# archi-physics/archi

Measured on AMD Instinct MI355X. Metric: kNN queries/sec @ top-10, 10M x 768 bf16 corpus, higher is better.
Workload: dtype bf16

## Files before the change

### archi_amd/csrc/index.hip

```cpp
#include "index.h"
#include "switches.h"

#include <algorithm>
#include <atomic>
#include <cmath>
#include <cstring>
#include <limits>
#include <chrono>
#include <dlfcn.h>
#include <unordered_set>

namespace ak {

static thread_local std::string g_err;
void set_error(const std::string &msg) { g_err = msg; }

extern "C" char **environ;
static const std::unordered_map<std::string, std::string> &env_snapshot() {
    static const std::unordered_map<std::string, std::string> *snap = [] {
        auto *m = new std::unordered_map<std::string, std::string>();
        for (char **e = environ; e && *e; e++) {
            if (strncmp(*e, "AK_", 3) != 0) continue;
            const char *eq = strchr(*e, '=');
            if (eq) (*m)[std::string(*e, (size_t)(eq - *e))] = std::string(eq + 1);
        }
        return m;
    }();
    return *snap;
}
const char *env_get(const char *name) {
    const auto &m = env_snapshot();
    const auto it = m.find(name);
    return it == m.end() ? nullptr : it->second.c_str();
}
int env_int(const char *name, int dflt) {
    const char *e = env_get(name);
    return e && *e ? atoi(e) : dflt;
}
namespace {
struct SwitchName { const char *name; std::atomic<int> Switches::*field; int dflt; bool is_flag; bool wrong_results; bool is_char; };
const SwitchName g_switch_names[] = {
    {"AK_SCAN_CFG", &Switches::scan_cfg, 0, false, false, true},
    {"AK_SCAN_MFMA", &Switches::scan_mfma, 0, false, false, false},
    {"AK_SCAN_I8", &Switches::scan_i8, AK_SCAN_I8_DEFAULT, false, false, false},
    {"AK_SCAN_BLOCKS", &Switches::scan_blocks, 0, false, false, false},
    {"AK_SCAN_NO192", &Switches::scan_no192, 0, true, false, false},
    {"AK_SEED_RATIO", &Switches::seed_ratio, 32, false, false, false},
    {"AK_SEED_DIV", &Switches::seed_div, 0, false, false, false},
    {"AK_PRE_DIV", &Switches::pre_div, 0, false, false, false},
    {"AK_SCAN_NOSEED", &Switches::scan_noseed, 0, true, false, false},
    {"AK_SCAN_NOPRE", &Switches::scan_nopre, 0, true, false, false},
    {"AK_TAIL_OLD", &Switches::tail_old, 0, true, false, false},
    {"AK_RERANK_OLD", &Switches::rerank_old, 0, false, false, false},
    {"AK_SCAN_DBG", &Switches::scan_dbg, 0, true, false, false},
    {"AK_COALESCE_STATS", &Switches::coalesce_stats, 0, true, false, false},
    {"AK_COALESCE", &Switches::coalesce, 1, false, false, false},
    {"AK_LEX_BATCH_PAIRS", &Switches::lex_batch_pairs, 1 << 24, false, false, false},
    {"AK_LEX_BATCH_TERMS", &Switches::lex_batch_terms, 0, false, false, false},
    {"AK_SHARD_INJECT", &Switches::shard_inject, 0, false, false, false},
    {"AK_QUERY_FUSED", &Switches::query_fused, 0, false, false, false},
#if AK_DBG_KERNELS
    {"AK_SCAN_ABLATE", &Switches::scan_ablate, 0, false, true, false},
    {"AK_TAIL_ABLATE", &Switches::tail_ablate, 0, false, true, false},
#endif
};
int switch_value(const SwitchName &n, const char *v) {
    if (!v || !*v) return n.dflt;
    if (n.is_char) return (int)(unsigned char)v[0];
    if (n.is_flag) return 1;
    return atoi(v);
}
}
Switches &switches() {
    static Switches sw;
    static const bool once = [] {
        for (const SwitchName &n : g_switch_names) {
            if (n.wrong_results && !DBG_KERNELS) continue;
            (sw.*(n.field)).store(switch_value(n, env_get(n.name)), std::memory_order_relaxed);
        }
        if (const char *e = env_get("AK_SCAN_R192")) sw.scan_r192_pm.store((int)(atof(e) * 1000.0 + 0.5), std::memory_order_relaxed);
        return true;
    }();
    (void)once;
    return sw;
}
__attribute__((constructor)) static void ak_read_environment_at_load() { (void)switches(); }
int switches_set(const char *name, const char *value) {
    if (!name) return -1;
    Switches &sw = switches();
    if (!strcmp(name, "AK_SCAN_R192")) {
        sw.scan_r192_pm.store(value && *value ? (int)(atof(value) * 1000.0 + 0.5) : 850, std::memory_order_relaxed);
        return 0;
    }
    for (const SwitchName &n : g_switch_names)
        if (!strcmp(name, n.name)) {
            if (n.wrong_results && !DBG_KERNELS) return -1;
            if (!DBG_KERNELS && n.is_char && value && (*value == 'X' || *value == 'O')) return -1;
            if (!DBG_KERNELS && n.field == &Switches::scan_mfma && switch_value(n, value) != 0) return -1;
            if (n.field == &Switches::scan_mfma && switch_value(n, value) != 0 && switch_value(n, value) != 16 && switch_value(n, value) != 32) return -1;
            (sw.*(n.field)).store(switch_value(n, value), std::memory_order_relaxed);
            return 0;
        }
    return -1;
}

namespace {
struct RoctxApi {
    int (*push)(const char *) = nullptr;
    int (*pop)() = nullptr;
    RoctxApi() {
        for (const char *lib : {"librocprofiler-sdk-roctx.so.1", "librocprofiler-sdk-roctx.so", "libroctx64.so.4", "libroctx64.so"}) {
            if (void *h = dlopen(lib, RTLD_NOW | RTLD_GLOBAL)) {
                push = (int (*)(const char *))dlsym(h, "roctxRangePushA");
                pop = (int (*)())dlsym(h, "roctxRangePop");
                if (push && pop) return;
                push = nullptr; pop = nullptr;
            }
        }
    }
};
const RoctxApi &roctx() {
    static const RoctxApi api;
    return api;
}
}
RoctxRange::RoctxRange(const char *name) : on(roctx().push != nullptr) { if (on) roctx().push(name); }
RoctxRange::~RoctxRange() { if (on) roctx().pop(); }

int Workspace::reserve(size_t need) {
    if (need <= bytes) return 0;
    if (buf) hipFree(buf);
    buf = nullptr; bytes = 0;
    AK_HIP(hipMalloc(&buf, need));
    bytes = need;
    return 0;
}
void Workspace::release() {
    if (buf) hipFree(buf);
    buf = nullptr; bytes = 0;
}

constexpr size_t SCRATCH_KEEP = 256ull << 20;
struct ThreadCtx {
    hipStream_t stream = nullptr;
    char *dev = nullptr; size_t dev_cap = 0;
    char *ws = nullptr; size_t ws_cap = 0;
    char *pin = nullptr; size_t pin_cap = 0;
    void trim() {
        if (dev_cap > SCRATCH_KEEP) { hipFree(dev); dev = nullptr; dev_cap = 0; }
        if (ws_cap > SCRATCH_KEEP) { hipFree(ws); ws = nullptr; ws_cap = 0; }
        if (pin_cap > SCRATCH_KEEP) { hipHostFree(pin); pin = nullptr; pin_cap = 0; }
    }
// ... 1235 lines not shown
```

### archi_amd/csrc/scan.hip

```cpp
#include <atomic>
#include "index.h"
#include "switches.h"
#include "mfma_tile.h"

#include <type_traits>

namespace ak {
using namespace mt;

constexpr int BK = 64;

__device__ inline uint64_t ld_sc1(const uint64_t *p) { return __builtin_nontemporal_load(p); }

__device__ inline float max3f(float a, float b, float c) {
    float r;
    asm("v_max3_f32 %0, %1, %2, %3" : "=v"(r) : "v"(a), "v"(b), "v"(c));
    return r;
}
__device__ inline float max3z(float a, float b) {
    float r;
    asm("v_max3_f32 %0, %1, %2, 0" : "=v"(r) : "v"(a), "v"(b));
    return r;
}

// ... 67 lines not shown

template <int NS>
__device__ __noinline__ int compact_impl(uint64_t *buf, int m, int k, int limit, float mar, int lane,
                                          float *thr_io, int *cnt_out, int *trig_out, int trig_max,
                                          uint64_t *final_out ) {
    uint64_t key[NS];
#pragma unroll
    for (int j = 0; j < NS; j++) {
        const int idx = j * 64 + lane;
        key[j] = idx < m ? ld_sc1(buf + idx) : KEY_INVALID;
    }
    float thr = *thr_io;
    if (m >= k) {
        const uint64_t tk = kth_key<NS>(key, k);
        const float t = key_score((uint32_t)(tk >> 32)) - mar;
        if (t > thr) thr = t;
    }
    uint64_t cut = ((uint64_t)score_key(thr) << 32) | 0xffffffffull;
    int c = 0;
#pragma unroll
    for (int j = 0; j < NS; j++) c += __popcll(__ballot(key[j] != KEY_INVALID && key[j] <= cut));
    if (c > limit) cut = kth_key<NS>(key, limit);
    uint64_t *dst = final_out ? final_out : buf;
    int run = 0;
#pragma unroll
    for (int j = 0; j < NS; j++) {
        const bool keep = key[j] != KEY_INVALID && key[j] <= cut;
        const uint64_t mask = __ballot(keep);
        const int pos = run + __popcll(mask & ((1ull << lane) - 1ull));
        if (keep) dst[pos] = key[j];
        run += __popcll(mask);
    }
    if (final_out) {
        for (int i = run + lane; i < limit; i += 64) final_out[i] = KEY_INVALID;
    } else if (lane == 0) {
        *cnt_out = run;
        const int tr = 2 * run > 64 ? 2 * run : 64;
        *trig_out = tr < trig_max ? tr : trig_max;
    }
    if (lane == 0) *thr_io = thr;
    return run;
}

template <int CAP>
__device__ inline int compact_wave(uint64_t *buf, int m, int k, int limit, float mar, int lane, float *thr_io,
                                    int *cnt_out, int *trig_out, int trig_max, uint64_t *final_out) {
    if (m <= 64) return compact_impl<1>(buf, m, k, limit, mar, lane, thr_io, cnt_out, trig_out, trig_max, final_out);
    else if (m <= 128) return compact_impl<2>(buf, m, k, limit, mar, lane, thr_io, cnt_out, trig_out, trig_max, final_out);
    else if (m <= 256) return compact_impl<4>(buf, m, k, limit, mar, lane, thr_io, cnt_out, trig_out, trig_max, final_out);
    else if (CAP >= 512 && m <= 512) return compact_impl<8>(buf, m, k, limit, mar, lane, thr_io, cnt_out, trig_out, trig_max, final_out);
    else return compact_impl<CAP / 64>(buf, m, k, limit, mar, lane, thr_io, cnt_out, trig_out, trig_max, final_out);
}

template <int WM_, int WN_, int MI_, int NI_, int NSTAGE_, int MINW_, bool PHASED_ = false, int MFMA_ = 32>
struct ScanCfg {
    static constexpr int WM = WM_, WN = WN_, MI = MI_, NI = NI_, NSTAGE = NSTAGE_, MINW = MINW_;
    static constexpr bool PHASED = PHASED_;
    static constexpr int MFMA = MFMA_;
    static constexpr bool I8 = false;
    using Shape32 = ScanCfg<WM_, WN_, MI_, NI_, NSTAGE_, MINW_, PHASED_, 32>;
    static_assert(MFMA_ == 32 || (MFMA_ == 16 && PHASED_), "the 16x16x32 shape exists for the phased tiles");
    static constexpr int AHEAD = NSTAGE_ - 1;
    static constexpr int BKB = 128;
    static constexpr int RPP = 1024 / BKB;
    static constexpr int CPR = BKB / 16;
    static constexpr int NSUB = BKB / 32;
    static constexpr int NW = WM * WN;
    static constexpr int THREADS = NW * 64;
    static constexpr int BM = WM * MI * 32;
    static constexpr int BN = WN * NI * 32;
    static constexpr int A_BYTES = BM * BKB, B_BYTES = BN * BKB;
    static constexpr int A_PW = BM / RPP / NW;
    static constexpr int B_PW = BN / RPP / NW;
    static constexpr int LOADS = A_PW + B_PW;
    static constexpr int CAP = BM >= 256 ? 1024 : 512;
    static constexpr int LDS_BYTES = NSTAGE * (A_BYTES + B_BYTES) + (4 * BM + 4 * BN + 4 + 128) * 4;
    static constexpr bool SEED_GM_LDS = PHASED_ && MI_ * NI_ >= 8;
    static constexpr int SEED_LDS_BYTES = LDS_BYTES + (SEED_GM_LDS ? NW * MI_ * NI_ * 64 * 4 : 0);
    static_assert(SEED_LDS_BYTES <= 160 * 1024, "LDS budget");
    static_assert((BM / RPP) % NW == 0 && (BN / RPP) % NW == 0, "pieces must divide over the waves");
    static_assert(NSTAGE >= 2 && NSTAGE <= 4, "ring depth");
    static_assert(BM / 64 <= NW, "ea/eb staging uses one wave per 64 rows");
    static_assert(!PHASED_ || (NSTAGE_ == 2 && ((WM_ == 2 && WN_ == 4 && MI_ == 4 && (NI_ == 2 || NI_ == 1)) ||
                                                 (WM_ == 4 && WN_ == 2 && MI_ == 2 && NI_ == 3))),
                  "phased K-loop: 256 x 256 / 256 x 128 tile (8 waves of 128 x 64 / 128 x 32) or 256 x 192 (8 waves of 64 x 96), two K-tile buffers");
};

template <bool IS_BF16, class C, bool SEED, bool INSTR, bool SEEDPASS = false>
__global__ __launch_bounds__(C::THREADS, C::MINW) void k_scan(
    const uint16_t *__restrict__ rows, const float *__restrict__ ea, const float *__restrict__ eb,
    const float *__restrict__ gb, int64_t gb_blocks, const uint8_t *__restrict__ filter, int64_t row_begin, int64_t n, int D, const uint16_t *__restrict__ qs, int nq,
    int nslices, int nqg, int k, int kp, const float *__restrict__ thr0, const float *__restrict__ mar,
    int slice_off, int nslices_total, uint64_t *__restrict__ cand, uint64_t *__restrict__ out_c,
    float *__restrict__ thr_out, int flags_arg, long long *__restrict__ dbg_arg, int64_t sample_tiles, int tstride,
    int *__restrict__ dense_cnt, unsigned int *__restrict__ dense_thr) {
    constexpr int BM = C::BM, BN = C::BN, NW = C::NW, MI = C::MI, NI = C::NI, NSTAGE = C::NSTAGE, CAP = C::CAP;
    constexpr bool I8 = C::I8;
    constexpr int EB = I8 ? 1 : 2;
    static_assert(!I8 || (C::MFMA == 16 && C::PHASED && !SEED), "the int8 scan is the phased tile on the 16x16 shape; its pre-seeding stays on 16 bits");
    constexpr bool M16 = C::MFMA == 16;
    static_assert(!(M16 && SEED), "the pre-seeding launch runs the 32x32x16 shape (C::Shape32)");
    const int flags = INSTR ? flags_arg : 0;
    long long *const dbg = INSTR ? dbg_arg : nullptr;
    extern __shared__ __attribute__((aligned(16))) char smem[];
    char *sA = smem;
    char *sB = smem + NSTAGE * C::A_BYTES;
    float *s_ea = (float *)(smem + NSTAGE * (C::A_BYTES + C::B_BYTES));
    float *s_eb = s_ea + 2 * BM;
    float *s_thr = s_eb + 2 * BM;
    int *s_cnt = (int *)(s_thr + BN);
    float *s_mar = (float *)(s_cnt + BN);
    int *s_trig = (int *)(s_mar + BN);
    int *s_need = s_trig + BN;
    float *s_gb = (float *)(s_need + 4);
// ... 93 lines not shown
                if constexpr (INSTR) n_comp++;
                compact_wave<CAP>(my_cand + (size_t)q * CAP, m, k, CAP - 2 * BM, s_mar[q], lane, &s_thr[q], &s_cnt[q],
                                  &s_trig[q], CAP - 2 * BM, nullptr);
            }
        }
        wait_vm<0>();
        __syncthreads();
        if (tid == 0) *s_need = 0;
        __syncthreads();
    };

    auto tile_epilogue = [&](int t, int64_t tile_row0) {
        const int par = t & 1;
        const float *t_ea = s_ea + par * BM, *t_eb = s_eb + par * BM, *t_gb = s_gb + par * 64;
        const bool tail = tile_row0 + BM > n;
        const int rows_left = tail ? (int)(n - tile_row0) : BM;
        if constexpr (SEED) {
#pragma unroll
            for (int mi = 0; mi < MI; mi++) {
#pragma unroll
                for (int g = 0; g < 4; g++) {
                    const int base = (wr * MI + mi) * 32 + 8 * g + 4 * kh;
                    float4 e4 = *(const float4 *)&t_ea[base], b4 = *(const float4 *)&t_eb[base];
                    if (tail) {
                        float *pe = (float *)&e4, *pb = (float *)&b4;
#pragma unroll
                        for (int j = 0; j < 4; j++)
                            if (base + j >= rows_left) { pe[j] = 0.f; pb[j] = -__builtin_inff(); }
                    }
#pragma unroll
                    for (int ni = 0; ni < NI; ni++) {
                        const f32x16 &a = acc[mi][ni];
                        float &gmx = GM_LDS ? s_gmx[(mi * NI + ni) * 64] : gm[GM_LDS ? 0 : mi][GM_LDS ? 0 : ni];
                        gmx = fmaxf(fmaxf(gmx, fmaf(a[4 * g + 0], e4.x, b4.x)),
                                    fmaxf(fmaxf(fmaf(a[4 * g + 1], e4.y, b4.y), fmaf(a[4 * g + 2], e4.z, b4.z)),
                                          fmaf(a[4 * g + 3], e4.w, b4.w)));
                    }
                }
                __builtin_amdgcn_sched_barrier(0);
            }
            return;
        }
        if (INSTR && (flags & 1)) {
#pragma unroll
            for (int mi = 0; mi < MI; mi++)
#pragma unroll
                for (int ni = 0; ni < NI; ni++) keep_live(acc[mi][ni]);
            return;
        }
        if constexpr (M16) {
            int ln = lane;
            asm volatile("" : "+v"(ln));
            const int r16 = ln & 15, kq = ln >> 4;
#if !AK_DBG_KERNELS
            mfma_settle(acc);
#endif
#pragma unroll
            for (int mi = 0; mi < MI; mi++) {
                const float gea = t_gb[(wr * MI + mi) * 4 + (kq & 1)], geb = t_gb[(wr * MI + mi) * 4 + 2 + (kq & 1)];
#pragma unroll
                for (int ni = 0; ni < NI; ni++) {
                    const f32x16 &a = acc[mi][ni];
#pragma unroll
                    for (int c = 0; c < 2; c++) {
                        const int lo = 4 * c, hi = 8 + 4 * c;
                        const i32x16 ia = __builtin_bit_cast(i32x16, a);
                        auto imax = [](int x, int y) { return x > y ? x : y; };
                        float dpos;
                        if constexpr (I8) {
                            dpos = (float)imax(imax(imax(imax(ia[lo], ia[lo + 1]), imax(ia[lo + 2], ia[lo + 3])),
                                                    imax(imax(ia[hi], ia[hi + 1]), imax(ia[hi + 2], ia[hi + 3]))), 0);
                        } else {
#if AK_DBG_KERNELS
                            dpos = fmaxf(fmaxf(fmaxf(fmaxf(a[lo], a[lo + 1]), fmaxf(a[lo + 2], a[lo + 3])),
                                               fmaxf(fmaxf(a[hi], a[hi + 1]), fmaxf(a[hi + 2], a[hi + 3]))), 0.f);
#else
                            dpos = max3z(max3f(max3f(a[lo], a[lo + 1], a[lo + 2]), max3f(a[lo + 3], a[hi], a[hi + 1]), a[hi + 2]), a[hi + 3]);
#endif
                        }
                        const float U = fmaf(dpos, gea, geb);
                        const float thr = s_thr[(wc * NI + ni) * 32 + 16 * c + r16];
                        if (U >= thr && !(INSTR && (flags & 16))) {
                            if constexpr (INSTR) n_slow++;
                            float sc[8];
                            float mx = -__builtin_inff();
#pragma unroll
                            for (int h = 0; h < 2; h++) {
                                const int base = (wr * MI + mi) * 32 + 16 * h + 4 * kq;
                                float4 e4 = *(const float4 *)&t_ea[base], b4 = *(const float4 *)&t_eb[base];
                                if (tail) {
                                    float *pe = (float *)&e4, *pb = (float *)&b4;
#pragma unroll
                                    for (int j = 0; j < 4; j++)
                                        if (base + j >= rows_left) { pe[j] = 0.f; pb[j] = -__builtin_inff(); }
                                }
                                const int o = 8 * h + 4 * c;
                                const float d0 = I8 ? (float)ia[o + 0] : a[o + 0], d1 = I8 ? (float)ia[o + 1] : a[o + 1],
                                            d2 = I8 ? (float)ia[o + 2] : a[o + 2], d3 = I8 ? (float)ia[o + 3] : a[o + 3];
                                sc[4 * h + 0] = fmaf(d0, e4.x, b4.x); sc[4 * h + 1] = fmaf(d1, e4.y, b4.y);
                                sc[4 * h + 2] = fmaf(d2, e4.z, b4.z); sc[4 * h + 3] = fmaf(d3, e4.w, b4.w);
                                mx = fmaxf(fmaxf(mx, sc[4 * h + 0]), fmaxf(fmaxf(sc[4 * h + 1], sc[4 * h + 2]), sc[4 * h + 3]));
                            }
                            if (mx >= thr) {
                                const int qcol = (wc * NI + ni) * 32 + 16 * c + r16;
                                int nh = 0;
#pragma unroll
                                for (int e = 0; e < 8; e++) nh += sc[e] >= thr ? 1 : 0;
                                int pos = atomicAdd(&s_cnt[qcol], nh);
                                if (pos + nh > s_trig[qcol]) *s_need = 1;
                                uint64_t *dstq = my_cand + (size_t)qcol * CAP;
                                const uint32_t rbase = (uint32_t)(tile_row0 + (wr * MI + mi) * 32 + 4 * kq);
#pragma unroll
                                for (int e = 0; e < 8; e++) {
                                    if (sc[e] >= thr) {
                                        dstq[pos] = ((uint64_t)score_key(sc[e]) << 32) | (uint64_t)(rbase + (e & 3) + 16 * (e >> 2));
                                        pos++;
                                    }
                                }
                            }
                        }
                    }
                }
            }
            return;
        }
        float thr_q[NI];
#pragma unroll
        for (int ni = 0; ni < NI; ni++) thr_q[ni] = s_thr[(wc * NI + ni) * 32 + r];
#if !AK_DBG_KERNELS
        mfma_settle(acc);
#endif
#pragma unroll
        for (int mi = 0; mi < MI; mi++) {
            const float gea = t_gb[(wr * MI + mi) * 4 + kh], geb = t_gb[(wr * MI + mi) * 4 + 2 + kh];
#pragma unroll
            for (int ni = 0; ni < NI; ni++) {
                const f32x16 &a = acc[mi][ni];
#if AK_DBG_KERNELS
                const float m01 = fmaxf(fmaxf(a[0], a[1]), fmaxf(a[2], a[3])), m23 = fmaxf(fmaxf(a[4], a[5]), fmaxf(a[6], a[7])),
                            m45 = fmaxf(fmaxf(a[8], a[9]), fmaxf(a[10], a[11])), m67 = fmaxf(fmaxf(a[12], a[13]), fmaxf(a[14], a[15]));
                const float dmax = fmaxf(fmaxf(m01, m23), fmaxf(m45, m67));
                const float dpos = fmaxf(dmax, 0.f);
#else
                const float dpos = max3z(max3f(max3f(a[0], a[1], a[2]), max3f(a[3], a[4], a[5]), max3f(a[6], a[7], a[8])),
                                         max3f(max3f(a[9], a[10], a[11]), max3f(a[12], a[13], a[14]), a[15]));
#endif
                const float U = fmaf(dpos, gea, geb);
                const float thr = thr_q[ni];
                if (U >= thr && !(INSTR && (flags & 16))) {
                    if constexpr (INSTR) n_slow++;
                    float sc[16];
                    float mx = -__builtin_inff();
#pragma unroll
                    for (int g = 0; g < 4; g++) {
                        const int base = (wr * MI + mi) * 32 + 8 * g + 4 * kh;
                        float4 e4 = *(const float4 *)&t_ea[base], b4 = *(const float4 *)&t_eb[base];
                        if (tail) {
                            float *pe = (float *)&e4, *pb = (float *)&b4;
#pragma unroll
                            for (int j = 0; j < 4; j++)
                                if (base + j >= rows_left) { pe[j] = 0.f; pb[j] = -__builtin_inff(); }
                        }
                        sc[4 * g + 0] = fmaf(a[4 * g + 0], e4.x, b4.x); sc[4 * g + 1] = fmaf(a[4 * g + 1], e4.y, b4.y);
                        sc[4 * g + 2] = fmaf(a[4 * g + 2], e4.z, b4.z); sc[4 * g + 3] = fmaf(a[4 * g + 3], e4.w, b4.w);
                        mx = fmaxf(fmaxf(mx, sc[4 * g + 0]), fmaxf(fmaxf(sc[4 * g + 1], sc[4 * g + 2]), sc[4 * g + 3]));
                    }
                    if (mx >= thr) {
                        const int qcol = (wc * NI + ni) * 32 + r;
                        int nh = 0;
#pragma unroll
                        for (int e = 0; e < 16; e++) nh += sc[e] >= thr ? 1 : 0;
                        int pos = atomicAdd(&s_cnt[qcol], nh);
                        if (pos + nh > s_trig[qcol]) *s_need = 1;
// ... 818 lines not shown
        for (int off = 32; off >= 1; off >>= 1) {
            const uint64_t k2 = __shfl_xor(bk, off);
            const int64_t i2 = __shfl_xor(bi, off);
            if (k2 < bk || (k2 == bk && i2 < bi)) { bk = k2; bi = i2; }
        }
        const bool valid = bk != KEY_INVALID;
        const double d = valid ? key_dist(bk) : __builtin_nan("");
        if (lane == 0) {
            out_ids[(int64_t)qi * k + round] = valid ? bi : -1;
            out_dist[(int64_t)qi * k + round] = d;
        }
        if (!valid) {
            for (int r2 = round + 1 + lane; r2 < k; r2 += 64) {
                out_ids[(int64_t)qi * k + r2] = -1;
                out_dist[(int64_t)qi * k + r2] = __builtin_nan("");
            }
            break;
        }
        cnt++; dk = d;
#pragma unroll
        for (int j = 0; j < NS; j++)
            if (ek[j] == bk && ei[j] == bi) { ek[j] = KEY_INVALID; ei[j] = INT64_MAX; }
    }
    float smin = -__builtin_inff();
    for (int j = lane; j < nslots; j += 64) {
        const float t = thr_slots[(int64_t)qi * nslots + j];
        if (t > -3.0e38f) smin = fmaxf(smin, t);
    }
#pragma unroll
    for (int off = 32; off >= 1; off >>= 1) smin = fmaxf(smin, __shfl_xor(smin, off));
    if (lane != 0) return;
    if (out_cnt) out_cnt[qi] = cnt;
    int ok = 0;
    const float nbq = nb[qi];
    const bool qfinite = nbq > 0.f && nbq < __builtin_inff();
    if (cnt == k && qfinite && dk == dk) {
        const QPrep p = prep[qi];
        if (valid_c == kp) smin = fmaxf(smin, key_score((uint32_t)(last_c >> 32)));
        if (smin == -__builtin_inff()) ok = 1;
        else {
            const double bound = p.a * (double)smin + p.b + p.eps;
            double t;
            if (metric == AK_METRIC_COSINE) t = 1.0 - dk;
            else if (metric == AK_METRIC_IP) t = -dk;
            else t = -dk * dk;
            ok = t > bound;
        }
    }
    cert[qi] = ok;
    if (stats) atomicAdd((unsigned long long *)&stats[2], (unsigned long long)valid_c);
}

constexpr int SHIP_P = 16, SHIP_Q = 16, SHIP_R = 16;
template <int S> using CfgPs = ScanCfg<2, 4, 4, 2, 2, 2, true, S>;
template <int S> using CfgQs = ScanCfg<2, 4, 4, 1, 2, 2, true, S>;
template <int S> using CfgRs = ScanCfg<4, 2, 2, 3, 2, 2, true, S>;
using CfgP = CfgPs<SHIP_P>;
using CfgQ = CfgQs<SHIP_Q>;
using CfgX = ScanCfg<2, 4, 4, 2, 2, 2>;
using CfgL = ScanCfg<4, 2, 2, 2, 3, 2>;
using CfgM = ScanCfg<4, 1, 2, 2, 3, 1>;
using CfgS = ScanCfg<4, 1, 2, 1, 3, 1>;
using CfgO = ScanCfg<2, 2, 2, 2, 2, 2>;
struct CfgP8 : CfgPs<16> { static constexpr bool I8 = true; };
using CfgR = CfgRs<SHIP_R>;

struct CfgInfo { int bm, bn, cap, threads, lds, blocks_per_cu; };
template <class C> constexpr CfgInfo info_of(int bpc) { return CfgInfo{C::BM, C::BN, C::CAP, C::THREADS, C::LDS_BYTES, bpc}; }
static const CfgInfo g_cfgs[8] = {info_of<CfgL>(1), info_of<CfgM>(1), info_of<CfgS>(1), info_of<CfgO>(2), info_of<CfgX>(1), info_of<CfgP>(1), info_of<CfgQ>(1),
                                  info_of<CfgR>(1)};
enum { CFG_L = 0, CFG_M = 1, CFG_S = 2, CFG_O = 3, CFG_X = 4, CFG_P = 5, CFG_Q = 6, CFG_R = 7 };
#if AK_DBG_KERNELS
#define AK_SCAN_XO_CASES(SCAN, R0, R1, NS, THR, SOFF, DBG, SP)            \
        case CFG_X: SCAN(CfgX, R0, R1, NS, THR, SOFF, DBG, SP); break;    \
        case CFG_O: SCAN(CfgO, R0, R1, NS, THR, SOFF, DBG, SP); break;
#else
#define AK_SCAN_XO_CASES(SCAN, R0, R1, NS, THR, SOFF, DBG, SP)
#endif

static bool big_shard(const Index &ix) { return ix.dim >= 768 && (ix.n + 255) / 256 >= 4096; }

static int pick_cfg(int nq, const Index &ix) {
    if (const int forced = switches().scan_cfg.load(std::memory_order_relaxed)) {
        switch (forced) { case 'L': return CFG_L; case 'M': return CFG_M; case 'S': return CFG_S;
                        case 'O': if (DBG_KERNELS) return CFG_O; break;
                        case 'X': if (DBG_KERNELS) return CFG_X; break;
                        case 'P': return ix.dim < 128 ? CFG_L : CFG_P; case 'Q': return ix.dim < 128 ? CFG_L : CFG_Q;
                        case 'R': return ix.dim < 128 ? CFG_L : CFG_R; }
    }
    if (nq <= 32) return CFG_S;
    if (nq <= 64) return CFG_M;
    if (nq <= 128) return CFG_L;
    if (ix.dim < 128) return CFG_L;
    const int g128 = (nq + 127) / 128, g192 = (nq + 191) / 192, g256 = (nq + 255) / 256;
    const bool big = big_shard(ix);
    const double r192 = switches().scan_r192_pm.load(std::memory_order_relaxed) * 1e-3;
    const bool no192 = switches().scan_no192.load(std::memory_order_relaxed) != 0;
    const double cp = g256, cr = no192 ? 1e9 : g192 * r192, cq = g128 * 0.62;
    if (big) {
        if (cr < cp && cr < cq) return CFG_R;
        return cp <= cq ? CFG_P : CFG_Q;
    }
    const int base = nq <= 256 ? CFG_Q : (g256 * 1.62 < g128 ? CFG_P : CFG_Q);
    return cr < (base == CFG_P ? cp : cq) ? CFG_R : base;
}

constexpr int I8_KP = 512;

bool fast_supported(const Index &ix, int nq, int k) {
    if (ix.dim % BK != 0) return false;
    if (ix.n < 4096) return false;
    if (k > 128) return false;
    return nq > 0;
}

static inline size_t al(size_t x) { return (x + 255) & ~(size_t)255; }

FastPlan fast_plan(const Index &ix, int nq, int k, bool widest, bool allow_i8) {
// ... 143 lines not shown
    uint64_t *top_k = (uint64_t *)p; p += al((size_t)nq * kp * 8);
    int64_t *top_i = (int64_t *)p; p += al((size_t)nq * kp * 8);
    uint64_t *rr_k = (uint64_t *)p; p += al((size_t)nq * kp * 8);
    int64_t *rr_i = (int64_t *)p; p += al((size_t)nq * kp * 8);
    int64_t *fin_i = (int64_t *)p; p += al((size_t)nq * k * 8);
    double *fin_d = (double *)p; p += al((size_t)nq * k * 8);
    const bool i8 = plan.i8 != 0;
    int8_t *qs8 = nullptr; QPrep *prep8 = nullptr; float *mar8 = nullptr, *thr_fin = nullptr; int *sd_cnt = nullptr, *sd_cert = nullptr;
    if (i8) {
        qs8 = (int8_t *)p; p += al((size_t)nq_pad * ix.dim);
        prep8 = (QPrep *)p; p += al((size_t)nq * sizeof(QPrep));
        mar8 = (float *)p; p += al((size_t)nq * 4);
        thr_fin = (float *)p; p += al((size_t)nq * 4);
        sd_cnt = (int *)p; p += al((size_t)nq * 4);
        sd_cert = (int *)p; p += al((size_t)nq * 4);
        if (plan.cfg != CFG_P || kp != I8_KP) AK_FAIL(-1, "fast_search: the int8 plan is tile P with k' = 512");
    }
    void *scratch = p;

    const bool dense = i8 || (kp == TAIL_KP && ix.dim <= TAIL_MAX_DIM && !switches().tail_old.load(std::memory_order_relaxed));
    int *dcnt = dense ? d_cnt : nullptr;
    unsigned int *dthr = dense ? d_thr : nullptr;

    const bool bf = ix.dtype != AK_DTYPE_F16;
    const int shadowed = ix.dtype == AK_DTYPE_F32;
    if (bf) k_query_setup<true><<<nq_pad, 64, 0, st>>>(queries_dev, nb_dev, nb_ready ? 0 : 1, nq, nq_pad, ix.dim, ix.metric, ix.max_na,
                                                       shadowed ? ix.max_rho : 0.f, qs, prep, mar, stats_dev, dcnt, dthr);
    else k_query_setup<false><<<nq_pad, 64, 0, st>>>(queries_dev, nb_dev, nb_ready ? 0 : 1, nq, nq_pad, ix.dim, ix.metric, ix.max_na, 0.f,
                                                     qs, prep, mar, stats_dev, dcnt, dthr);
    if (i8) k_query_setup8<<<nq_pad, 64, 0, st>>>(queries_dev, nb_dev, nq, ix.dim, ix.metric, ix.max_na, ix.max_rho8, qs8, prep8, mar8);
    AK_HIP(hipGetLastError());

    hipEvent_t ev0 = nullptr, ev1 = nullptr;
    std::unique_lock<std::mutex> prof_lk(ix.prof_mu, std::defer_lock);
    const bool want_dbg = switches().scan_dbg.load(std::memory_order_relaxed) != 0;
    if (ix.profile || want_dbg) prof_lk.lock();
    if (ix.profile) {
        if (ix.prof_used == ix.prof_events.size()) {
            hipEvent_t a, b;
            AK_HIP(hipEventCreate(&a));
            AK_HIP(hipEventCreate(&b));
            ix.prof_events.emplace_back(a, b);
        }
        ev0 = ix.prof_events[ix.prof_used].first;
        ev1 = ix.prof_events[ix.prof_used].second;
        ix.prof_used++;
    }
    int rc = 0;
#define SCAN(CFG, R0, R1, NS, THR, SOFF, DBG, SP)                                                                    \
    rc = bf ? launch_scan<true, CFG, false, SP>(ix, filter_dev, R0, R1, qs, nq, NS, nqg, k, kp, THR, mar, SOFF, ns_tot, cand, out_c, thr_slots, DBG, st, 0, 1, dcnt, dthr) \
            : launch_scan<false, CFG, false, SP>(ix, filter_dev, R0, R1, qs, nq, NS, nqg, k, kp, THR, mar, SOFF, ns_tot, cand, out_c, thr_slots, DBG, st, 0, 1, dcnt, dthr)
#if AK_DBG_KERNELS
    const int mfma_forced = switches().scan_mfma.load(std::memory_order_relaxed);
#define SCAN_SHAPED(T, SHIPPED, R0, R1, NS, THR, SOFF, DBG, SP)                         \
    if (mfma_forced == 16) { SCAN(T<16>, R0, R1, NS, THR, SOFF, DBG, SP); }             \
    else if (mfma_forced == 32) { SCAN(T<32>, R0, R1, NS, THR, SOFF, DBG, SP); }        \
    else { SCAN(SHIPPED, R0, R1, NS, THR, SOFF, DBG, SP); }
#else
#define SCAN_SHAPED(T, SHIPPED, R0, R1, NS, THR, SOFF, DBG, SP) SCAN(SHIPPED, R0, R1, NS, THR, SOFF, DBG, SP)
#endif
#define SCAN_ANY(R0, R1, NS, THR, SOFF, DBG, SP)                         \
    switch (plan.cfg) {                                          \
        case CFG_L: SCAN(CfgL, R0, R1, NS, THR, SOFF, DBG, SP); break;    \
        case CFG_M: SCAN(CfgM, R0, R1, NS, THR, SOFF, DBG, SP); break;    \
        case CFG_S: SCAN(CfgS, R0, R1, NS, THR, SOFF, DBG, SP); break;    \
        AK_SCAN_XO_CASES(SCAN, R0, R1, NS, THR, SOFF, DBG, SP)            \
        case CFG_P: SCAN_SHAPED(CfgPs, CfgP, R0, R1, NS, THR, SOFF, DBG, SP); break;    \
        case CFG_Q: SCAN_SHAPED(CfgQs, CfgQ, R0, R1, NS, THR, SOFF, DBG, SP); break;    \
        case CFG_R: SCAN_SHAPED(CfgRs, CfgR, R0, R1, NS, THR, SOFF, DBG, SP); break;    \
        default: AK_FAIL(-1, "scan: tile configuration not in this library (X and O: libarchi_hip_dbg.so)"); \
    }
#define SCAN8(R0, R1, NS, THR, SOFF, DBG, SP)                                                                                     \
    rc = launch_scan<true, CfgP8, false, SP>(ix, filter_dev, R0, R1, (const uint16_t *)qs8, nq, NS, nqg, k, kp, THR, mar8, SOFF, ns_tot, \
                                             cand, out_c, thr_slots, DBG, st, 0, 1, dcnt, dthr)
    long long *dbg0 = nullptr, *dbg1 = nullptr;
    if (want_dbg) {
        if (!ix.dbg_dev) { AK_HIP(hipMalloc((void **)&ix.dbg_dev, 2 * 65536 * 8)); }
        AK_HIP(hipMemsetAsync(ix.dbg_dev, 0, 2 * 65536 * 8, st));
        dbg0 = ix.dbg_dev; dbg1 = ix.dbg_dev + 65536;
    }
    const float *thr_main = nullptr;
    const float *thr_seed = nullptr;
    {
        if (plan.pre_tiles > 0) {
#define PRE(CFG)                                                                                                          \
    rc = bf ? launch_scan<true, CFG, true>(ix, filter_dev, 0, ix.n, qs, nq, plan.pre_slices, nqg, k, kp, nullptr, mar, 0, 0, \
                                           nullptr, nullptr, gmax, nullptr, st, plan.pre_tiles, plan.pre_stride)         \
            : launch_scan<false, CFG, true>(ix, filter_dev, 0, ix.n, qs, nq, plan.pre_slices, nqg, k, kp, nullptr, mar, 0, 0, \
                                            nullptr, nullptr, gmax, nullptr, st, plan.pre_tiles, plan.pre_stride)
            switch (plan.cfg) {
                case CFG_L: PRE(CfgL); break;
                case CFG_M: PRE(CfgM); break;
                case CFG_S: PRE(CfgS); break;
#if AK_DBG_KERNELS
                case CFG_X: PRE(CfgX); break;
                case CFG_O: PRE(CfgO); break;
#endif
                case CFG_P: PRE(CfgP::Shape32); break;
                case CFG_Q: PRE(CfgQ::Shape32); break;
                case CFG_R: PRE(CfgR::Shape32); break;
                default: AK_FAIL(-1, "scan: tile configuration not in this library (X and O: libarchi_hip_dbg.so)");
            }
#undef PRE
            if (rc) return rc;
            k_seed_kth<<<nq, 64, 0, st>>>(gmax, plan.pre_slices * (c.bm / 16), prep, k, thr0);
            if (i8) k_thr_to_i8<<<(nq + 63) / 64, 64, 0, st>>>(prep, prep8, nq, thr0);
            AK_HIP(hipGetLastError());
            thr_seed = thr0;
            thr_main = thr0;
        }
    }
    if (nss > 0 && i8) {
        SCAN8(0, plan.seed_rows, nss, thr_seed, 0, dbg0, true);
        if (rc) return rc;
        rc = fused_tail(ix, queries_dev, nb_dev, nq, k, out_c, (int64_t)ns_tot * kp, d_cnt, d_thr, thr_seed, prep8, fin_i, fin_d, sd_cnt,
                        sd_cert, nullptr, st);
        if (rc) return rc;
        k_seed_exact_thr<<<(nq + 63) / 64, 64, 0, st>>>(fin_d, sd_cnt, prep8, nq, k, ix.metric, thr_seed != nullptr, thr0);
        AK_HIP(hipGetLastError());
        thr_main = thr0;
    } else if (nss > 0) {
        SCAN_ANY(0, plan.seed_rows, nss, thr_seed, 0, dbg0, true);
        if (rc) return rc;
        const int64_t seed_in = (int64_t)nss * kp, seed_stride = (int64_t)ns_tot * kp;
#define KTH(EPT)                                                                                                         \
    do {                                                                                                                 \
        if (thr_seed) k_seed_kth_lists<EPT, true><<<nq, 256, 0, st>>>(out_c, seed_in, seed_stride, prep, k, thr0, dcnt);   \
        else k_seed_kth_lists<EPT, false><<<nq, 256, 0, st>>>(out_c, seed_in, seed_stride, prep, k, thr0, dcnt);           \
    } while (0)
        if (seed_in <= 16 * 256) KTH(16);
        else if (seed_in <= 32 * 256) KTH(32);
        else if (seed_in <= 64 * 256) KTH(64);
        else {
            if (dense) AK_FAIL(-1, "fast_search: dense lists with more than 16384 seed candidates");
            rc = select_topk_strided(out_c, nq, seed_in, seed_stride, k, top_k, top_i, scratch, st);
            if (rc) return rc;
            if (thr_seed) k_seed_thr<true><<<(nq + 63) / 64, 64, 0, st>>>(top_k, prep, nq, k, k, thr0);
            else k_seed_thr<false><<<(nq + 63) / 64, 64, 0, st>>>(top_k, prep, nq, k, k, thr0);
        }
#undef KTH
        AK_HIP(hipGetLastError());
        thr_main = thr0;
    }
    if (ev0) AK_HIP(hipEventRecord(ev0, st));
    if (i8) { SCAN8(plan.seed_rows, ix.n, ns, thr_main, nss, dbg1, false); }
    else { SCAN_ANY(plan.seed_rows, ix.n, ns, thr_main, nss, dbg1, false); }
#undef SCAN8
#undef SCAN_ANY
#undef SCAN_SHAPED
#undef SCAN
    if (rc) return rc;
    if (ev1) AK_HIP(hipEventRecord(ev1, st));

    if (i8) {
        ix.s8_searches.fetch_add(1, std::memory_order_relaxed);
        k_select_dense<<<nq, SD_THREADS, 0, st>>>(out_c, (int64_t)ns_tot * kp, d_cnt, d_thr, thr_main, kp, top_k, thr_fin);
        AK_HIP(hipGetLastError());
        rc = rerank(ix, queries_dev, nb_dev, nq, kp, top_k, rr_k, rr_i, st);
        if (rc) return rc;
        k_finalize<8><<<nq, 64, 0, st>>>(top_k, rr_k, rr_i, prep8, nb_dev, thr_fin, 1, k, kp, ix.metric, out_ids_dev, out_dist_dev,
                                         out_cnt_dev, cert_dev, stats_dev);
        AK_HIP(hipGetLastError());
        return 0;
    }
    if (dense)
        return fused_tail(ix, queries_dev, nb_dev, nq, k, out_c, (int64_t)ns_tot * kp, d_cnt, d_thr, thr_main, prep, out_ids_dev,
                          out_dist_dev, out_cnt_dev, cert_dev, stats_dev, st);
    rc = select_keys_topk(out_c, nq, (int64_t)ns_tot * kp, (int64_t)ns_tot * kp, kp, top_k, scratch, st);
    if (rc) return rc;
    rc = rerank(ix, queries_dev, nb_dev, nq, kp, top_k, rr_k, rr_i, st);
    if (rc) return rc;
#define FIN(NS) k_finalize<NS><<<nq, 64, 0, st>>>(top_k, rr_k, rr_i, prep, nb_dev, thr_slots, ns_tot, k, kp, ix.metric, out_ids_dev, \
                                              out_dist_dev, out_cnt_dev, cert_dev, stats_dev)
    if (kp <= 64) FIN(1); else if (kp <= 128) FIN(2); else if (kp <= 256) FIN(4); else FIN(8);
#undef FIN
    AK_HIP(hipGetLastError());
    return 0;
}

}
```

### archi_amd/csrc/switches.h

```cpp
#pragma once
#include <atomic>

#include "common.h"

namespace ak {

constexpr int AK_SCAN_I8_DEFAULT = 1;

struct Switches {
    std::atomic<int> scan_cfg{0};
    std::atomic<int> scan_mfma{0};
    std::atomic<int> scan_i8{AK_SCAN_I8_DEFAULT};
    std::atomic<int> scan_blocks{0};
    std::atomic<int> scan_r192_pm{850};
    std::atomic<int> scan_no192{0};
    std::atomic<int> seed_ratio{32};
    std::atomic<int> seed_div{0};
    std::atomic<int> pre_div{0};
    std::atomic<int> scan_noseed{0};
    std::atomic<int> scan_nopre{0};
    std::atomic<int> tail_old{0};
    std::atomic<int> rerank_old{0};
    std::atomic<int> scan_dbg{0};
    std::atomic<int> coalesce_stats{0};
    std::atomic<int> query_fused{0};
    std::atomic<int> coalesce{1};
    std::atomic<int> lex_batch_pairs{1 << 24};
    std::atomic<int> lex_batch_terms{0};
    std::atomic<int> shard_inject{0};
    std::atomic<int> scan_ablate{0};
    std::atomic<int> tail_ablate{0};
};
Switches &switches();
int switches_set(const char *name, const char *value);
const char *env_get(const char *name);
int env_int(const char *name, int dflt);
inline int dbg_env_int(const char *name, int dflt) { return DBG_KERNELS ? env_int(name, dflt) : dflt; }

}
```

Baseline: 126,400.

## Add whole-tile exact-score filter path for int8 16x16 scan tiles

Adds a FILT=1 variant of the scan epilogue that computes exact per-row scores for every site up front, packs the pass/fail result into a hit bitmask, and only runs the append path for sites that pass. This replaces the per-site bound check followed by a branchy slow path. Because int8 is on by default and CfgP8 now ships with FILT=1, the default int8 scan uses this path. The trade-off is unconditional FMA work and LDS row-term loads on every tile, in exchange for less warp divergence and no false-positive slow-path entries. The epilogue code is also reorganized into lambdas, and a debug switch is added to force the filter on or off.

Result: faster. 131,000, median of 6 (+3.6%).

```diff
diff --git a/archi_amd/csrc/index.hip b/archi_amd/csrc/index.hip
--- a/archi_amd/csrc/index.hip
+++ b/archi_amd/csrc/index.hip
@@ -42,6 +42,7 @@
 const SwitchName g_switch_names[] = {
     {"AK_SCAN_CFG", &Switches::scan_cfg, 0, false, false, true},
     {"AK_SCAN_MFMA", &Switches::scan_mfma, 0, false, false, false},
+    {"AK_SCAN_FILTER", &Switches::scan_filter, 0, false, false, false},
     {"AK_SCAN_I8", &Switches::scan_i8, AK_SCAN_I8_DEFAULT, false, false, false},
     {"AK_SCAN_BLOCKS", &Switches::scan_blocks, 0, false, false, false},
     {"AK_SCAN_NO192", &Switches::scan_no192, 0, true, false, false},
@@ -98,6 +99,8 @@
             if (!DBG_KERNELS && n.is_char && value && (*value == 'X' || *value == 'O')) return -1;
             if (!DBG_KERNELS && n.field == &Switches::scan_mfma && switch_value(n, value) != 0) return -1;
             if (n.field == &Switches::scan_mfma && switch_value(n, value) != 0 && switch_value(n, value) != 16 && switch_value(n, value) != 32) return -1;
+            if (!DBG_KERNELS && n.field == &Switches::scan_filter && switch_value(n, value) != 0) return -1;
+            if (n.field == &Switches::scan_filter && (switch_value(n, value) < 0 || switch_value(n, value) > 2)) return -1;
             (sw.*(n.field)).store(switch_value(n, value), std::memory_order_relaxed);
             return 0;
         }
diff --git a/archi_amd/csrc/scan.hip b/archi_amd/csrc/scan.hip
--- a/archi_amd/csrc/scan.hip
+++ b/archi_amd/csrc/scan.hip
@@ -143,14 +143,16 @@
     else return compact_impl<CAP / 64>(buf, m, k, limit, mar, lane, thr_io, cnt_out, trig_out, trig_max, final_out);
 }
 
-template <int WM_, int WN_, int MI_, int NI_, int NSTAGE_, int MINW_, bool PHASED_ = false, int MFMA_ = 32>
+template <int WM_, int WN_, int MI_, int NI_, int NSTAGE_, int MINW_, bool PHASED_ = false, int FILT_ = 0, int MFMA_ = 32>
 struct ScanCfg {
     static constexpr int WM = WM_, WN = WN_, MI = MI_, NI = NI_, NSTAGE = NSTAGE_, MINW = MINW_;
     static constexpr bool PHASED = PHASED_;
     static constexpr int MFMA = MFMA_;
+    static constexpr int FILT = FILT_;
     static constexpr bool I8 = false;
-    using Shape32 = ScanCfg<WM_, WN_, MI_, NI_, NSTAGE_, MINW_, PHASED_, 32>;
+    using Shape32 = ScanCfg<WM_, WN_, MI_, NI_, NSTAGE_, MINW_, PHASED_, 0, 32>;
     static_assert(MFMA_ == 32 || (MFMA_ == 16 && PHASED_), "the 16x16x32 shape exists for the phased tiles");
+    static_assert(FILT_ == 0 || (FILT_ == 1 && MFMA_ == 16), "the whole-tile filter exists for the 16x16x32 tiles");
     static constexpr int AHEAD = NSTAGE_ - 1;
     static constexpr int BKB = 128;
     static constexpr int RPP = 1024 / BKB;
@@ -350,6 +352,131 @@
             int ln = lane;
             asm volatile("" : "+v"(ln));
             const int r16 = ln & 15, kq = ln >> 4;
+            auto imax = [](int x, int y) { return x > y ? x : y; };
+            auto site_dpos = [&](int mi, int ni, int c) -> float {
+                const f32x16 &a = acc[mi][ni];
+                const int lo = 4 * c, hi = 8 + 4 * c;
+                if constexpr (I8) {
+                    const i32x16 ia = __builtin_bit_cast(i32x16, a);
+                    return (float)imax(imax(imax(imax(ia[lo], ia[lo + 1]), imax(ia[lo + 2], ia[lo + 3])),
+                                            imax(imax(ia[hi], ia[hi + 1]), imax(ia[hi + 2], ia[hi + 3]))), 0);
+                } else {
+#if AK_DBG_KERNELS
+                    return fmaxf(fmaxf(fmaxf(fmaxf(a[lo], a[lo + 1]), fmaxf(a[lo + 2], a[lo + 3])),
+                                       fmaxf(fmaxf(a[hi], a[hi + 1]), fmaxf(a[hi + 2], a[hi + 3]))), 0.f);
+#else
+                    return max3z(max3f(max3f(a[lo], a[lo + 1], a[lo + 2]), max3f(a[lo + 3], a[hi], a[hi + 1]), a[hi + 2]), a[hi + 3]);
+#endif
+                }
+            };
+            auto row_terms = [&](int mi, float4 (&e4)[2], float4 (&b4)[2]) {
+#pragma unroll
+                for (int h = 0; h < 2; h++) {
+                    const int base = (wr * MI + mi) * 32 + 16 * h + 4 * kq;
+                    e4[h] = *(const float4 *)&t_ea[base];
+                    b4[h] = *(const float4 *)&t_eb[base];
+                    if (tail) {
+                        float *pe = (float *)&e4[h], *pb = (float *)&b4[h];
+#pragma unroll
+                        for (int j = 0; j < 4; j++)
+                            if (base + j >= rows_left) { pe[j] = 0.f; pb[j] = -__builtin_inff(); }
+                    }
+                }
+            };
+            auto site_scores = [&](int mi, int ni, int c, const float4 (&e4s)[2], const float4 (&b4s)[2], float (&sc)[8]) -> float {
+                const f32x16 &a = acc[mi][ni];
+                const i32x16 ia = __builtin_bit_cast(i32x16, a);
+                float mx = -__builtin_inff();
+#pragma unroll
+                for (int h = 0; h < 2; h++) {
+                    const float4 e4 = e4s[h], b4 = b4s[h];
+                    const int o = 8 * h + 4 * c;
+                    const float d0 = I8 ? (float)ia[o + 0] : a[o + 0], d1 = I8 ? (float)ia[o + 1] : a[o + 1],
+                                d2 = I8 ? (float)ia[o + 2] : a[o + 2], d3 = I8 ? (float)ia[o + 3] : a[o + 3];
+                    sc[4 * h + 0] = fmaf(d0, e4.x, b4.x); sc[4 * h + 1] = fmaf(d1, e4.y, b4.y);
+                    sc[4 * h + 2] = fmaf(d2, e4.z, b4.z); sc[4 * h + 3] = fmaf(d3, e4.w, b4.w);
+                    mx = fmaxf(fmaxf(mx, sc[4 * h + 0]), fmaxf(fmaxf(sc[4 * h + 1], sc[4 * h + 2]), sc[4 * h + 3]));
+                }
+                return mx;
+            };
+            auto site_append = [&](int mi, int ni, int c, float thr, const float (&sc)[8]) {
+                if (INSTR && (flags & 64)) return;
+                const int qcol = (wc * NI + ni) * 32 + 16 * c + r16;
+                int nh = 0;
+#pragma unroll
+                for (int e = 0; e < 8; e++) nh += sc[e] >= thr ? 1 : 0;
+                int pos = atomicAdd(&s_cnt[qcol], nh);
+                if (pos + nh > s_trig[qcol]) *s_need = 1;
+                uint64_t *dstq = my_cand + (size_t)qcol * CAP;
+                const uint32_t rbase = (uint32_t)(tile_row0 + (wr * MI + mi) * 32 + 4 * kq);
+#pragma unroll
+                for (int e = 0; e < 8; e++) {
+                    if (sc[e] >= thr) {
+                        dstq[pos] = ((uint64_t)score_key(sc[e]) << 32) | (uint64_t)(rbase + (e & 3) + 16 * (e >> 2));
+                        pos++;
+                    }
+                }
+            };
+            if constexpr (C::FILT == 1) {
+                static_assert(2 * MI * NI <= 32, "one hit bit per site");
+                constexpr int TG = (!I8 && MI * NI >= 8) ? 2 : MI;
+                float4 e4[TG][2], b4[TG][2];
+                float thr_s[NI][2];
+#pragma unroll
+                for (int ni = 0; ni < NI; ni++)
+#pragma unroll
+                    for (int c = 0; c < 2; c++) thr_s[ni][c] = s_thr[(wc * NI + ni) * 32 + 16 * c + r16];
+                uint32_t hits = 0;
+#pragma unroll
+                for (int g = 0; g < MI / TG; g++) {
+#pragma unroll
+                    for (int j = 0; j < TG; j++) row_terms(g * TG + j, e4[j], b4[j]);
+#pragma unroll
+                    for (int j = 0; j < TG; j++)
+#pragma unroll
+                        for (int ni = 0; ni < NI; ni++)
+#pragma unroll
+                            for (int c = 0; c < 2; c++) {
+                                float sc[8];
+                                const int mi = g * TG + j;
+                                hits |= site_scores(mi, ni, c, e4[j], b4[j], sc) >= thr_s[ni][c] ? 1u << ((mi * NI + ni) * 2 + c) : 0u;
+                            }
+                    if (MI / TG > 1) __builtin_amdgcn_sched_barrier(0);
+                }
+                if (INSTR && (flags & 16)) hits = 0;
+                if (hits) {
+#pragma unroll
+                    for (int g = 0; g < MI / TG; g++) {
+                        if (MI / TG > 1) {
+                            if (!(hits & (((1u << (2 * NI * TG)) - 1u) << (g * TG * NI * 2)))) continue;
+#pragma unroll
+                            for (int j = 0; j < TG; j++) row_terms(g * TG + j, e4[j], b4[j]);
+                        }
+#pragma unroll
+                        for (int j = 0; j < TG; j++)
+#pragma unroll
+                            for (int ni = 0; ni < NI; ni++)
+#pragma unroll
+                                for (int c = 0; c < 2; c++) {
+                                    const int mi = g * TG + j;
+                                    if (hits & (1u << ((mi * NI + ni) * 2 + c))) {
+                                        if constexpr (INSTR) n_slow++;
+                                        float sc[8];
+                                        site_scores(mi, ni, c, e4[j], b4[j], sc);
+                                        site_append(mi, ni, c, thr_s[ni][c], sc);
+                                    }
+                                }
+                    }
+                }
+                return;
+            }
+            auto site_slow = [&](int mi, int ni, int c, float thr) {
+                if constexpr (INSTR) n_slow++;
+                float4 e4[2], b4[2];
+                row_terms(mi, e4, b4);
+                float sc[8];
+                if (site_scores(mi, ni, c, e4, b4, sc) >= thr) site_append(mi, ni, c, thr, sc);
+            };
 #if !AK_DBG_KERNELS
             mfma_settle(acc);
 #endif
@@ -358,65 +485,11 @@
                 const float gea = t_gb[(wr * MI + mi) * 4 + (kq & 1)], geb = t_gb[(wr * MI + mi) * 4 + 2 + (kq & 1)];
 #pragma unroll
                 for (int ni = 0; ni < NI; ni++) {
-                    const f32x16 &a = acc[mi][ni];
 #pragma unroll
                     for (int c = 0; c < 2; c++) {
-                        const int lo = 4 * c, hi = 8 + 4 * c;
-                        const i32x16 ia = __builtin_bit_cast(i32x16, a);
-                        auto imax = [](int x, int y) { return x > y ? x : y; };
-                        float dpos;
-                        if constexpr (I8) {
-                            dpos = (float)imax(imax(imax(imax(ia[lo], ia[lo + 1]), imax(ia[lo + 2], ia[lo + 3])),
-                                                    imax(imax(ia[hi], ia[hi + 1]), imax(ia[hi + 2], ia[hi + 3]))), 0);
-                        } else {
-#if AK_DBG_KERNELS
-                            dpos = fmaxf(fmaxf(fmaxf(fmaxf(a[lo], a[lo + 1]), fmaxf(a[lo + 2], a[lo + 3])),
-                                               fmaxf(fmaxf(a[hi], a[hi + 1]), fmaxf(a[hi + 2], a[hi + 3]))), 0.f);
-#else
-                            dpos = max3z(max3f(max3f(a[lo], a[lo + 1], a[lo + 2]), max3f(a[lo + 3], a[hi], a[hi + 1]), a[hi + 2]), a[hi + 3]);
-#endif
-                        }
-                        const float U = fmaf(dpos, gea, geb);
+                        const float U = fmaf(site_dpos(mi, ni, c), gea, geb);
                         const float thr = s_thr[(wc * NI + ni) * 32 + 16 * c + r16];
-                        if (U >= thr && !(INSTR && (flags & 16))) {
-                            if constexpr (INSTR) n_slow++;
-                            float sc[8];
-                            float mx = -__builtin_inff();
-#pragma unroll
-                            for (int h = 0; h < 2; h++) {
-                                const int base = (wr * MI + mi) * 32 + 16 * h + 4 * kq;
-                                float4 e4 = *(const float4 *)&t_ea[base], b4 = *(const float4 *)&t_eb[base];
-                                if (tail) {
-                                    float *pe = (float *)&e4, *pb = (float *)&b4;
-#pragma unroll
-                                    for (int j = 0; j < 4; j++)
-                                        if (base + j >= rows_left) { pe[j] = 0.f; pb[j] = -__builtin_inff(); }
-                                }
-                                const int o = 8 * h + 4 * c;
-                                const float d0 = I8 ? (float)ia[o + 0] : a[o + 0], d1 = I8 ? (float)ia[o + 1] : a[o + 1],
-                                            d2 = I8 ? (float)ia[o + 2] : a[o + 2], d3 = I8 ? (float)ia[o + 3] : a[o + 3];
-                                sc[4 * h + 0] = fmaf(d0, e4.x, b4.x); sc[4 * h + 1] = fmaf(d1, e4.y, b4.y);
-                                sc[4 * h + 2] = fmaf(d2, e4.z, b4.z); sc[4 * h + 3] = fmaf(d3, e4.w, b4.w);
-                                mx = fmaxf(fmaxf(mx, sc[4 * h + 0]), fmaxf(fmaxf(sc[4 * h + 1], sc[4 * h + 2]), sc[4 * h + 3]));
-                            }
-                            if (mx >= thr) {
-                                const int qcol = (wc * NI + ni) * 32 + 16 * c + r16;
-                                int nh = 0;
-#pragma unroll
-                                for (int e = 0; e < 8; e++) nh += sc[e] >= thr ? 1 : 0;
-                                int pos = atomicAdd(&s_cnt[qcol], nh);
-                                if (pos + nh > s_trig[qcol]) *s_need = 1;
-                                uint64_t *dstq = my_cand + (size_t)qcol * CAP;
-                                const uint32_t rbase = (uint32_t)(tile_row0 + (wr * MI + mi) * 32 + 4 * kq);
-#pragma unroll
-                                for (int e = 0; e < 8; e++) {
-                                    if (sc[e] >= thr) {
-                                        dstq[pos] = ((uint64_t)score_key(sc[e]) << 32) | (uint64_t)(rbase + (e & 3) + 16 * (e >> 2));
-                                        pos++;
-                                    }
-                                }
-                            }
-                        }
+                        if (U >= thr && !(INSTR && (flags & 16))) site_slow(mi, ni, c, thr);
                     }
                 }
             }
@@ -1341,18 +1414,20 @@
 }
 
 constexpr int SHIP_P = 16, SHIP_Q = 16, SHIP_R = 16;
-template <int S> using CfgPs = ScanCfg<2, 4, 4, 2, 2, 2, true, S>;
-template <int S> using CfgQs = ScanCfg<2, 4, 4, 1, 2, 2, true, S>;
-template <int S> using CfgRs = ScanCfg<4, 2, 2, 3, 2, 2, true, S>;
-using CfgP = CfgPs<SHIP_P>;
-using CfgQ = CfgQs<SHIP_Q>;
+constexpr int SHIP_FILT_P = 0, SHIP_FILT_P8 = 1, SHIP_FILT_Q = 0, SHIP_FILT_R = 0;
+template <int S, int F = 0> using CfgPs = ScanCfg<2, 4, 4, 2, 2, 2, true, S == 16 ? F : 0, S>;
+template <int S, int F = 0> using CfgQs = ScanCfg<2, 4, 4, 1, 2, 2, true, S == 16 ? F : 0, S>;
+template <int S, int F = 0> using CfgRs = ScanCfg<4, 2, 2, 3, 2, 2, true, S == 16 ? F : 0, S>;
+using CfgP = CfgPs<SHIP_P, SHIP_FILT_P>;
+using CfgQ = CfgQs<SHIP_Q, SHIP_FILT_Q>;
 using CfgX = ScanCfg<2, 4, 4, 2, 2, 2>;
 using CfgL = ScanCfg<4, 2, 2, 2, 3, 2>;
 using CfgM = ScanCfg<4, 1, 2, 2, 3, 1>;
 using CfgS = ScanCfg<4, 1, 2, 1, 3, 1>;
 using CfgO = ScanCfg<2, 2, 2, 2, 2, 2>;
-struct CfgP8 : CfgPs<16> { static constexpr bool I8 = true; };
-using CfgR = CfgRs<SHIP_R>;
+struct CfgP8 : CfgPs<16, SHIP_FILT_P8> { static constexpr bool I8 = true; };
+struct CfgP8f : CfgPs<16, 1 - SHIP_FILT_P8> { static constexpr bool I8 = true; };
+using CfgR = CfgRs<SHIP_R, SHIP_FILT_R>;
 
 struct CfgInfo { int bm, bn, cap, threads, lds, blocks_per_cu; };
 template <class C> constexpr CfgInfo info_of(int bpc) { return CfgInfo{C::BM, C::BN, C::CAP, C::THREADS, C::LDS_BYTES, bpc}; }
@@ -1602,10 +1677,11 @@
             : launch_scan<false, CFG, false, SP>(ix, filter_dev, R0, R1, qs, nq, NS, nqg, k, kp, THR, mar, SOFF, ns_tot, cand, out_c, thr_slots, DBG, st, 0, 1, dcnt, dthr)
 #if AK_DBG_KERNELS
     const int mfma_forced = switches().scan_mfma.load(std::memory_order_relaxed);
-#define SCAN_SHAPED(T, SHIPPED, R0, R1, NS, THR, SOFF, DBG, SP)                         \
-    if (mfma_forced == 16) { SCAN(T<16>, R0, R1, NS, THR, SOFF, DBG, SP); }             \
-    else if (mfma_forced == 32) { SCAN(T<32>, R0, R1, NS, THR, SOFF, DBG, SP); }        \
-    else { SCAN(SHIPPED, R0, R1, NS, THR, SOFF, DBG, SP); }
+    const int filt_forced = switches().scan_filter.load(std::memory_order_relaxed) - 1;
+#define SCAN_SHAPED(T, SHIPPED, R0, R1, NS, THR, SOFF, DBG, SP)                                                                  \
+    if ((mfma_forced ? mfma_forced : SHIPPED::MFMA) == 32) { using C_ = T<32>; SCAN(C_, R0, R1, NS, THR, SOFF, DBG, SP); }          \
+    else if ((filt_forced < 0 ? SHIPPED::FILT : filt_forced) == 1) { using C_ = T<16, 1>; SCAN(C_, R0, R1, NS, THR, SOFF, DBG, SP); } \
+    else { using C_ = T<16, 0>; SCAN(C_, R0, R1, NS, THR, SOFF, DBG, SP); }
 #else
 #define SCAN_SHAPED(T, SHIPPED, R0, R1, NS, THR, SOFF, DBG, SP) SCAN(SHIPPED, R0, R1, NS, THR, SOFF, DBG, SP)
 #endif
@@ -1620,9 +1696,16 @@
         case CFG_R: SCAN_SHAPED(CfgRs, CfgR, R0, R1, NS, THR, SOFF, DBG, SP); break;    \
         default: AK_FAIL(-1, "scan: tile configuration not in this library (X and O: libarchi_hip_dbg.so)"); \
     }
-#define SCAN8(R0, R1, NS, THR, SOFF, DBG, SP)                                                                                     \
-    rc = launch_scan<true, CfgP8, false, SP>(ix, filter_dev, R0, R1, (const uint16_t *)qs8, nq, NS, nqg, k, kp, THR, mar8, SOFF, ns_tot, \
-                                             cand, out_c, thr_slots, DBG, st, 0, 1, dcnt, dthr)
+#define SCAN8_T(T, R0, R1, NS, THR, SOFF, DBG, SP)                                                                                \
+    rc = launch_scan<true, T, false, SP>(ix, filter_dev, R0, R1, (const uint16_t *)qs8, nq, NS, nqg, k, kp, THR, mar8, SOFF, ns_tot, \
+                                         cand, out_c, thr_slots, DBG, st, 0, 1, dcnt, dthr)
+#if AK_DBG_KERNELS
+#define SCAN8(R0, R1, NS, THR, SOFF, DBG, SP)                                                                  \
+    if (filt_forced >= 0 && filt_forced != CfgP8::FILT) { SCAN8_T(CfgP8f, R0, R1, NS, THR, SOFF, DBG, SP); }   \
+    else { SCAN8_T(CfgP8, R0, R1, NS, THR, SOFF, DBG, SP); }
+#else
+#define SCAN8(R0, R1, NS, THR, SOFF, DBG, SP) SCAN8_T(CfgP8, R0, R1, NS, THR, SOFF, DBG, SP)
+#endif
     long long *dbg0 = nullptr, *dbg1 = nullptr;
     if (want_dbg) {
         if (!ix.dbg_dev) { AK_HIP(hipMalloc((void **)&ix.dbg_dev, 2 * 65536 * 8)); }
@@ -1696,6 +1779,7 @@
     if (i8) { SCAN8(plan.seed_rows, ix.n, ns, thr_main, nss, dbg1, false); }
     else { SCAN_ANY(plan.seed_rows, ix.n, ns, thr_main, nss, dbg1, false); }
 #undef SCAN8
+#undef SCAN8_T
 #undef SCAN_ANY
 #undef SCAN_SHAPED
 #undef SCAN
diff --git a/archi_amd/csrc/switches.h b/archi_amd/csrc/switches.h
--- a/archi_amd/csrc/switches.h
+++ b/archi_amd/csrc/switches.h
@@ -10,6 +10,7 @@
 struct Switches {
     std::atomic<int> scan_cfg{0};
     std::atomic<int> scan_mfma{0};
+    std::atomic<int> scan_filter{0};
     std::atomic<int> scan_i8{AK_SCAN_I8_DEFAULT};
     std::atomic<int> scan_blocks{0};
     std::atomic<int> scan_r192_pm{850};
```
